# eldenpark/halo2-pse

Measured on AMD Instinct MI355X. Metric: bn254_msm_g1_adds_per_sec, higher is better.
Workload: dtype u32x8 (256-bit Montgomery integers)

## Files before the change

halo2-pse_amd/csrc/api.hip:

```cpp
#include <dlfcn.h>
#include <rccl/rccl.h>
#include <stdarg.h>
#include <stdlib.h>
#include <string.h>

#include <atomic>
#include <condition_variable>
#include <deque>
#include <functional>
#include <shared_mutex>
#include <thread>

#include "../../include/halo2hip.h"
#include "../../include/halo2hip_debug.h"
#include "engine.h"

extern "C" {
static void lazy_forget(const void* key);
static void lazy_reset();
static void lazy_pin_consider(const uint64_t* bases_xy, size_t n);
}

namespace h2 {

int gen_scalars_device(uint64_t seed, uint64_t start, size_t n, Fe* d_out, hipStream_t s);
int gen_points_device(uint64_t seed, uint64_t start, size_t n, Affine* d_out, hipStream_t s);
void msm_set_window(uint32_t c);
void msm_set_max_chunk(size_t m);
void msm_set_stream(uint32_t chunks, double ratio, size_t min_n);
size_t msm_debug_ladder(size_t n, uint32_t chunks, double ratio, bool with_bases, size_t* out, size_t cap);
void msm_set_heavy_div(size_t d);
void msm_set_bin_entries(size_t d);
void msm_set_split_records(bool on);
void msm_set_bucket_order(int local);
void msm_set_quad_tail(bool on);
void msm_set_split_buckets(bool on);
void msm_set_plane_tail(bool on);
void ecfft_set_quad(bool on);
void ecfft_set_lazy(bool on);
void msm_set_fuse_limits(size_t entries, size_t max_n);
void msm_set_rowcol(uint64_t lanes, uint32_t flavour);
void ntt_set_smax(uint32_t v);
void ntt_set_two_pass(uint32_t lo, uint32_t hi);
void ntt_set_full_twiddle_budget(uint64_t bytes);
void ntt_set_batch_bytes(uint64_t bytes);
void ntt_set_two_pass_log_j(int v);
void ntt_set_full_max_log_m(uint32_t v);
void ntt_set_fold_tables(bool on);
void ntt_set_two_pass_batch_wgs(uint64_t v);
void msm_set_reserved_cus(uint32_t k);
uint32_t msm_get_reserved_cus();
uint32_t msm_get_window(size_t n);

static thread_local char g_err[512] = "";

void set_error(const char* fmt, ...) {
    va_list ap;
    va_start(ap, fmt);
    vsnprintf(g_err, sizeof(g_err), fmt, ap);
    va_end(ap);
}

int DevBuf::ensure(size_t bytes) {
    if (bytes <= cap) return 0;
    if (p) {
        H2_CHECK(hipDeviceSynchronize());
        H2_CHECK(hipFree(p));
        p = nullptr;
        cap = 0;
    }
    size_t want = bytes + bytes / 8 + 4096;
    hipError_t e = hipMalloc(&p, want);
    if (e != hipSuccess) {
        p = nullptr;
        set_error("hipMalloc(%zu) failed: %s", want, hipGetErrorString(e));
        return H2HIP_ENOMEM;
    }
    cap = want;
    return 0;
}

int HostBuf::ensure(size_t bytes) {
    if (bytes <= cap) return 0;
    if (p) {
        H2_CHECK(hipDeviceSynchronize());
        H2_CHECK(hipHostFree(p));
        p = nullptr;
        cap = 0;
    }
    size_t want = bytes * 2 + 4096;
    hipError_t e = hipHostMalloc(&p, want, hipHostMallocDefault);
    if (e != hipSuccess) {
        p = nullptr;
        set_error("hipHostMalloc(%zu) failed: %s", want, hipGetErrorString(e));
        return H2HIP_ENOMEM;
    }
    cap = want;
    return 0;
}

void HostBuf::release() {
    if (p) (void)hipHostFree(p);
    p = nullptr;
    cap = 0;
}

void DevBuf::release() {
    if (p) (void)hipFree(p);
    p = nullptr;
    cap = 0;
}

static std::shared_mutex g_engine_mu;
static Ctx g_ctx;
static std::vector<Ctx*> g_devs;
Ctx* ctx() { return &g_ctx; }
int n_devices() { return (int)g_devs.size(); }
Ctx* ctx_at(int i) { return g_devs[(size_t)i]; }

int Ctx::stage_h2d(void* d_dst, const void* h_src, size_t bytes, hipStream_t s) {
// ... 2060 lines not shown
    if (en.rc) return en.rc;
    return evaluate_h_host(en.c, desc, (uint64_t*)d_values, true, (hipStream_t)stream);
}

int h2hip_gen_scalars_device(uint64_t seed, uint64_t start, size_t n, void* d_out, void* stream) {
    if (n && !d_out) {
        set_error("gen_scalars: null output");
        return H2HIP_EINVAL;
    }
    Entry en("h2hip_gen_scalars_device", d_out);
    if (en.rc) return en.rc;
    return gen_scalars_device(seed, start, n, (Fe*)d_out, (hipStream_t)stream);
}

int h2hip_gen_points_device(uint64_t seed, uint64_t start, size_t n, void* d_out, void* stream) {
    if (n && !d_out) {
        set_error("gen_points: null output");
        return H2HIP_EINVAL;
    }
    Entry en("h2hip_gen_points_device", d_out);
    if (en.rc) return en.rc;
    return gen_points_device(seed, start, n, (Affine*)d_out, (hipStream_t)stream);
}

int h2hip_set_msm_window(uint32_t c) {
    if (c != 0 && (c < 2 || c > 24)) {
        set_error("msm window must be 0 (auto) or 2..24");
        return H2HIP_EINVAL;
    }
    msm_set_window(c);
    return 0;
}

uint32_t h2hip_get_msm_window(size_t n) { return msm_get_window(n); }
uint32_t h2hip_get_msm_window_fixed_base(size_t n) { return msm_table_window(n); }

int h2hip_debug_set_msm_max_chunk(size_t m) {
    msm_set_max_chunk(m);
    return 0;
}

int h2hip_debug_set_msm_stream(uint32_t chunks, uint32_t ratio_permille, size_t min_n) {
    msm_set_stream(chunks, ratio_permille / 1000.0, min_n);
    return 0;
}

size_t h2hip_debug_msm_stream_ladder(size_t n, uint32_t chunks, uint32_t ratio_permille, int with_bases, size_t* sizes, size_t cap) {
    if (!sizes && cap) return 0;
    return msm_debug_ladder(n, chunks, ratio_permille / 1000.0, with_bases != 0, sizes, cap);
}

int h2hip_debug_set_msm_heavy_div(size_t d) {
    msm_set_heavy_div(d);
    return 0;
}

int h2hip_debug_set_g2l_quad(int on) {
    ecfft_set_quad(on != 0);
    return 0;
}

int h2hip_debug_set_msm_fuse_limits(size_t entries, size_t max_n) {
    msm_set_fuse_limits(entries, max_n);
    return 0;
}

int h2hip_debug_set_msm_rowcol(uint64_t lanes, int use_asm) {
    msm_set_rowcol(lanes, (uint32_t)use_asm);
    return 0;
}

int h2hip_debug_set_msm_split_buckets(int on) {
    msm_set_split_buckets(on != 0);
    return 0;
}

int h2hip_debug_set_msm_plane_tail(int on) {
    Entry en;
    if (en.rc) return en.rc;
    msm_set_plane_tail(on != 0);
    return 0;
}

int h2hip_debug_set_msm_quad_tail(int on) {
    msm_set_quad_tail(on != 0);
    return 0;
}

int h2hip_debug_set_msm_bucket_order(int local) {
    msm_set_bucket_order(local);
    return 0;
}

int h2hip_debug_set_msm_split_records(int on) {
    msm_set_split_records(on != 0);
    return 0;
}

int h2hip_debug_set_msm_bin_entries(size_t d) {
    msm_set_bin_entries(d);
    return 0;
}

int h2hip_debug_set_evalh_max_local_slots(uint32_t v) {
    evalh_debug_set_max_local_slots(v);
    return 0;
}

int h2hip_debug_set_evalh_lookup_group_bytes(uint64_t v) {
    evalh_debug_set_lookup_group_bytes(v);
    return 0;
}

int h2hip_debug_evalh_program_muls(const h2hip_graph* g, uint32_t* n_mul) { return evalh_debug_program_muls(g, n_mul) ? H2HIP_EINVAL : 0; }

int h2hip_debug_set_evalh_codegen(int mode, uint32_t max_ops) {
    Entry en;
    if (en.rc) return en.rc;
    evalh_debug_set_codegen(mode, max_ops);
    return 0;
}

int h2hip_debug_evalh_codegen_source(const h2hip_graph* g, char* buf, size_t cap, size_t* len, int compile, double* seconds, size_t* code_bytes) {
    return evalh_debug_codegen_source(g, buf, cap, len, compile, seconds, code_bytes);
}

int h2hip_debug_evalh_codegen_stats(uint64_t out[5]) {
    if (!out) return H2HIP_EINVAL;
    evalh_debug_codegen_stats(out);
    return 0;
}

int h2hip_debug_evalh_compile_stats(const h2hip_graph* g, uint32_t* n_ops, uint32_t* n_slots) {
    return evalh_debug_compile_stats(g, n_ops, n_slots);
}

int h2hip_debug_set_msm_fuse_small(int on) {
    msm_set_fuse_small(on != 0);
    return 0;
}

int h2hip_debug_set_ntt_smax(uint32_t v) {
    ntt_set_smax(v);
    return 0;
}

int h2hip_debug_set_ntt_twiddle_budget(uint64_t bytes) {
    ntt_set_full_twiddle_budget(bytes);
    return 0;
}

int h2hip_debug_set_ntt_batch_bytes(uint64_t bytes) {
    ntt_set_batch_bytes(bytes);
    return 0;
}

int h2hip_debug_set_ntt_two_pass_batch_wgs(uint64_t v) {
    ntt_set_two_pass_batch_wgs(v);
    return 0;
}

int h2hip_debug_set_ntt_full_max_log_m(uint32_t v) {
    ntt_set_full_max_log_m(v);
    return 0;
}

// ... 59 lines not shown
```

halo2-pse_amd/csrc/msm.hip:

```cpp
#include <hip/hip_ext.h>
#include <string.h>

#include <atomic>
#include <condition_variable>
#include <thread>
#include <vector>

#include "ecq.h"
#include "engine.h"
#include "host64.h"

namespace h2 {

#define MSM_MAX_C1 1024u
#define MSM_MAX_L 12u
#define MSM_STAGE 16384u
#define MSM_COUNT_TILE 4096u

struct MsmPlan {
    uint32_t c;
    uint32_t W;
    uint32_t q;
    uint32_t cb;
    uint32_t NB;
// ... 759 lines not shown
    }
    if (role == 0) sh[quad] = acc;
    __syncthreads();
    for (uint32_t stride = G >> 1; stride >= 1; stride >>= 1) {
        if (g < stride) {
            XYZZu x = sh[quad];
            xyzzu_add_q(x, sh[quad + stride], role);
            if (role == 0) sh[quad] = x;
        }
        __syncthreads();
    }
    if (live && g == 0 && role == 0) J.out[task] = sh[quad];
}

__global__ void __launch_bounds__(64) msm_final_quad_kernel(FinalArgs args, uint32_t n_groups, XYZZu* __restrict__ partials, uint32_t* __restrict__ done,
                                                            XYZZ* __restrict__ set_sums) {
    __shared__ XYZZu sh[16];
    __shared__ uint32_t is_last;
    const uint32_t set = blockIdx.x / n_groups, group = blockIdx.x - set * n_groups;
    const uint32_t quad = threadIdx.x >> 2, role = threadIdx.x & 3;
    uint32_t e = group * 16 + quad;
    const XYZZu* base = nullptr;
    uint32_t stride = 0, o = 0, k = 0, nbits = 0;
    bool found = false;
#pragma unroll
    for (uint32_t i = 0; i < 4; i++) {
        if (i < args.n_arr && !found) {
            if (e < args.arr[i].len) {
                found = true;
                base = args.arr[i].base;
                stride = args.arr[i].stride;
                o = args.arr[i].o;
                k = args.arr[i].k;
                nbits = args.arr[i].nbits;
            } else {
                e -= args.arr[i].len;
            }
        }
    }
    XYZZu x = xyzzu_identity();
    if (found) {
        const uint32_t wgt = (e + o) << k;
        if (wgt) x = xyzzu_mul_small_q(base[(size_t)set * stride + e], wgt, nbits, role);
    }
    if (role == 0) sh[quad] = x;
    __syncthreads();
    for (uint32_t st = 8; st >= 1; st >>= 1) {
        if (quad < st) {
            XYZZu a = sh[quad];
            xyzzu_add_q(a, sh[quad + st], role);
            if (role == 0) sh[quad] = a;
        }
        __syncthreads();
    }
    if (n_groups == 1) {
        if (threadIdx.x == 0) set_sums[set] = xyzzu_to_ext(sh[0]);
        return;
    }
    if (threadIdx.x == 0) {
        partials[blockIdx.x] = sh[0];
        __threadfence();
        is_last = atomicAdd(&done[set], 1u) == n_groups - 1;
    }
    __syncthreads();
    if (!is_last) return;
    __builtin_amdgcn_fence(__ATOMIC_ACQUIRE, "agent");
    x = xyzzu_identity();
    if (quad < n_groups) x = partials[(size_t)set * n_groups + quad];
    if (role == 0) sh[quad] = x;
    __syncthreads();
    for (uint32_t st = 8; st >= 1; st >>= 1) {
        if (quad < st) {
            XYZZu a = sh[quad];
            xyzzu_add_q(a, sh[quad + st], role);
            if (role == 0) sh[quad] = a;
        }
        __syncthreads();
    }
    if (threadIdx.x == 0) set_sums[set] = xyzzu_to_ext(sh[0]);
}

#define MSM_PLANES_MAX 32
#define MSM_PLANE_SETS_MAX 4
struct PlaneJob {
    const XYZZu* base;
    uint32_t log_len;
    uint32_t o;
    uint32_t n_planes;
    uint32_t wgs;
    uint32_t first_plane;
    uint32_t first_block;
};
struct PlaneArgs {
    PlaneJob job[2];
    uint32_t blocks_per_set, planes_per_set;
};

__global__ void __launch_bounds__(256) msm_planes_kernel(PlaneArgs args, XYZZu* __restrict__ partials, uint32_t* __restrict__ done,
                                                         XYZZ* __restrict__ plane_sums) {
    __shared__ XYZZu sh[64];
    __shared__ uint32_t is_last;
    const uint32_t set = blockIdx.x / args.blocks_per_set, b = blockIdx.x - set * args.blocks_per_set;
    const PlaneJob& J = args.job[b >= args.job[1].first_block ? 1 : 0];
    const uint32_t pb = b - J.first_block, plane = pb / J.wgs, part = pb - plane * J.wgs;
    const XYZZu* X = J.base + ((size_t)set << J.log_len);
    const uint32_t quad = threadIdx.x >> 2, role = threadIdx.x & 3;
    const bool top = plane == J.log_len;
    const uint32_t count = top ? 1u : 1u << (J.log_len - 1);
    auto elem = [&](uint32_t t) -> XYZZu {
        if (t >= count) return xyzzu_identity();
        const uint32_t v = top ? (1u << J.log_len) : ((t >> plane) << (plane + 1)) | (1u << plane) | (t & ((1u << plane) - 1));
        return X[v - J.o];
    };
    const uint32_t t0 = part * 128 + 2 * quad;
    const XYZZu x = xyzzu_sum_q(elem(t0), elem(t0 + 1), role);
    if (role == 0) sh[quad] = x;
    __syncthreads();
    for (uint32_t st = 32; st >= 1; st >>= 1) {
        if (quad < st) {
            const XYZZu a = xyzzu_sum_q(sh[quad], sh[quad + st], role);
            if (role == 0) sh[quad] = a;
        }
        __syncthreads();
    }
    const uint32_t out = set * args.planes_per_set + J.first_plane + plane;
    if (J.wgs == 1) {
        if (threadIdx.x == 0) plane_sums[out] = xyzzu_to_ext(sh[0]);
        return;
    }
    if (threadIdx.x == 0) {
        partials[(size_t)out * 16 + part] = sh[0];
        __threadfence();
        is_last = atomicAdd(&done[out], 1u) == J.wgs - 1;
    }
    __syncthreads();
    if (!is_last) return;
    __builtin_amdgcn_fence(__ATOMIC_ACQUIRE, "agent");
    XYZZu y = xyzzu_identity();
    if (quad < J.wgs) y = partials[(size_t)out * 16 + quad];
    if (role == 0 && quad < 16) sh[quad] = y;
    __syncthreads();
    for (uint32_t st = 8; st >= 1; st >>= 1) {
        if (quad < st) {
            const XYZZu a = xyzzu_sum_q(sh[quad], sh[quad + st], role);
            if (role == 0) sh[quad] = a;
        }
        __syncthreads();
    }
    if (threadIdx.x == 0) plane_sums[out] = xyzzu_to_ext(sh[0]);
}

__global__ void __launch_bounds__(256) msm_table_step_kernel(const Affine* __restrict__ prev, XYZZ* __restrict__ out, uint32_t n, uint32_t c) {
    const uint32_t i = blockIdx.x * blockDim.x + threadIdx.x;
    if (i >= n) return;
    const Affine p = prev[i];
    if (affine_is_identity(p)) {
        out[i] = xyzz_identity();
        return;
    }
    XYZZu q = xyzzu_double_affine<FqUA>(fu_from_ext(p.x), fu_from_ext(p.y));
    for (uint32_t k = 1; k < c; k++) q = xyzzu_double(q);
    out[i] = xyzzu_to_ext(q);
}

static uint32_t g_window_override = 0;
static size_t g_heavy_div = 32768;
static size_t g_bin_entries = 8192;
static bool g_split_records = true;
void msm_set_split_records(bool on) { g_split_records = on; }
static uint64_t g_rowcol_lanes = 65536;
static bool g_rowcol_asm = true, g_rowcol_qtree = true;
void msm_set_rowcol(uint64_t lanes, uint32_t flavour) {
    g_rowcol_lanes = lanes ? lanes : 65536;
    g_rowcol_asm = flavour & 1;
    g_rowcol_qtree = flavour & 2;
}
static bool g_split_buckets = true;
void msm_set_split_buckets(bool on) { g_split_buckets = on; }
static bool g_quad_tail = true;
void msm_set_quad_tail(bool on) { g_quad_tail = on; }
static bool g_global_order = true;
void msm_set_bucket_order(int local) { g_global_order = local == 0; }
void msm_set_bin_entries(size_t d) { g_bin_entries = d ? d : 8192; }
void msm_set_heavy_div(size_t d) { g_heavy_div = d ? d : 32768; }
static size_t g_max_chunk = (size_t)1 << 26;
void msm_set_max_chunk(size_t m) { g_max_chunk = m ? m : ((size_t)1 << 26); }
static uint32_t g_reserved_cus = 0;
void msm_set_reserved_cus(uint32_t k) { g_reserved_cus = k; }
uint32_t msm_get_reserved_cus() { return g_reserved_cus; }
void msm_set_window(uint32_t c) { g_window_override = c; }

static uint32_t floor_log2(size_t n) {
    uint32_t lg = 0;
    while (((size_t)1 << (lg + 1)) <= n) lg++;
    return lg;
}

static uint32_t plain_window(size_t n, bool fused) {
    if (g_window_override) return g_window_override;
    const uint32_t lg = floor_log2(n);
    if (fused && lg >= 13 && lg <= 18) return lg <= 13 ? 10 : lg <= 16 ? 12 : lg == 17 ? 13 : 14;
    if (lg <= 8) return 7;
    if (lg <= 12) return 10;
    if (lg <= 14) return 13;
    if (lg <= 17) return 15;
    return 17;
}

static uint32_t normalise_window(uint32_t c) {
    if (c < 2) c = 2;
    if (c > 22) c = 22;
    const uint32_t W = (255 + c - 1) / c;
    return (255 + W - 1) / W;
}

uint32_t msm_table_window(size_t n) {
    if (g_window_override) return normalise_window(g_window_override);
    const uint32_t lg = floor_log2(n);
    uint32_t c = lg <= 12 ? 13 : lg <= 17 ? 17 : lg <= 21 ? 20 : 22;
    return normalise_window(c);
}

static MsmPlan make_plan(size_t n, bool fused, const MsmTable* tab, uint32_t force_c = 0) {
    MsmPlan p;
    uint32_t c = tab ? tab->c : force_c ? force_c : plain_window(n, fused);
    if (c < 2) c = 2;
    if (c > 24) c = 24;
    p.W = (255 + c - 1) / c;
    c = (255 + p.W - 1) / p.W;
    p.c = c;
    p.q = 255 - p.W * (c - 1);
    p.cb = c - 1;
// ... 200 lines not shown
        hipLaunchKernelGGL(msm_l2_kernel<true>, dim3(L.C1), dim3(1024), 0, s, (const uint2*)nullptr, (const uint32_t*)a.tmp_e, (const uint16_t*)a.tmp_k, cstart,
                           L.L, L.bin_shift, vals, start, counts, perm, g_global_order ? hist : (uint32_t*)nullptr);
    else
        hipLaunchKernelGGL(msm_l2_kernel<false>, dim3(L.C1), dim3(1024), 0, s, (const uint2*)(base + L.o_tmp), (const uint32_t*)nullptr,
                           (const uint16_t*)nullptr, cstart, L.L, L.bin_shift, vals, start, counts, perm, g_global_order ? hist : (uint32_t*)nullptr);
    H2_CHECK(hipGetLastError());
    hipLaunchKernelGGL(msm_bucket_scatter_kernel, dim3((L.K + 1024 * MSM_BS_PER - 1) / (1024 * MSM_BS_PER)), dim3(1024), 0, s, (const uint32_t*)counts,
                       (const uint32_t*)start, L.K, L.bin_shift, p.heavy_t, p.chunk, hist, g_global_order ? perm : (uint32_t*)nullptr,
                       (uint32_t*)(base + L.o_hcnt), (HeavyBucket*)(base + L.o_hb), (HeavyChunk*)(base + L.o_hc));
    H2_CHECK(hipGetLastError());
    c->timer_end(t1, s);
    return 0;
}

static int msm_stage_b(Ctx* c, const MsmLayout& L, char* base, const Affine* d_points, hipStream_t s, char* bbase = nullptr, bool cont = false,
                       bool combine = true) {
    const MsmPlan& p = L.p;
    if (!bbase) bbase = base;
    uint32_t* vals = (uint32_t*)(base + L.o_vals);
    uint32_t *start = (uint32_t*)(base + L.o_start), *counts = (uint32_t*)(base + L.o_counts), *perm = (uint32_t*)(base + L.o_perm);
    XYZZu* buckets = (XYZZu*)(bbase + L.o_buckets);
    uint32_t* hcnt = (uint32_t*)(base + L.o_hcnt);
    HeavyBucket* hb = (HeavyBucket*)(base + L.o_hb);
    HeavyChunk* hc = (HeavyChunk*)(base + L.o_hc);
    XYZZu* hs = (XYZZu*)(base + L.o_hs);
    int t2 = c->timer_begin("msm_accum", s);
    hipEvent_t ke0 = nullptr, ke1 = nullptr;
    XYZZu* parts = (XYZZu*)(bbase + L.o_parts);
    const uint32_t lanes = L.K << L.split_log;
    const uint32_t cont_u = cont ? 1u : 0u;
    const uint32_t hgrid = (uint32_t)(L.max_chunks < (size_t)c->sm_count ? L.max_chunks : (size_t)c->sm_count);
    const dim3 agrid(hgrid + (lanes + 255) / 256);
    if (c->timer_kernel("msm_accum", &ke0, &ke1) >= 0)
        hipExtLaunchKernelGGL(msm_accum_kernel, agrid, dim3(256), 0, s, ke0, ke1, 0, d_points, (const uint32_t*)vals, (const uint32_t*)start,
                              (const uint32_t*)counts, (const uint32_t*)perm, L.K, L.split_log, p.heavy_t, cont_u, parts, hgrid, (const uint32_t*)hcnt, hb,
                              (const HeavyChunk*)hc, hs);
    else
        hipLaunchKernelGGL(msm_accum_kernel, agrid, dim3(256), 0, s, d_points, (const uint32_t*)vals, (const uint32_t*)start, (const uint32_t*)counts,
                           (const uint32_t*)perm, L.K, L.split_log, p.heavy_t, cont_u, parts, hgrid, (const uint32_t*)hcnt, hb, (const HeavyChunk*)hc, hs);
    H2_CHECK(hipGetLastError());
    c->timer_end(t2, s);
    if (L.split_log && combine) {
        const uint32_t comb_lanes = L.K << (L.split_log - 1);
        hipLaunchKernelGGL(msm_combine_kernel, dim3((comb_lanes + 255) / 256), dim3(256), 0, s, (const XYZZu*)parts, L.K, L.split_log, buckets);
        H2_CHECK(hipGetLastError());
    }
    return 0;
}

static void rowcol_jobs(RowColArgs* ra, const XYZZu* in, XYZZu* out_rows, XYZZu* out_cols, uint32_t n_arr, uint32_t log_rows, uint32_t log_cols,
                        uint32_t* n_blocks, bool quad = false) {
    const uint64_t elems = (uint64_t)n_arr << (log_rows + log_cols);
    const uint64_t budget = (2 * elems) >> 4 > g_rowcol_lanes ? 2 * g_rowcol_lanes : g_rowcol_lanes;
    uint32_t t_log = 1;
    while (!quad && (2 * elems) >> t_log > budget) t_log++;
    for (uint32_t kind = 0; kind < 2; kind++) {
        RowColJob* j = &ra->job[ra->n_jobs++];
        const uint32_t log_terms = kind ? log_rows : log_cols, log_sums = kind ? log_cols : log_rows;
        uint32_t g_log = log_terms > t_log ? log_terms - t_log : 0;
        const uint32_t g_max = quad ? 4 : 8;
        if (g_log > g_max) g_log = g_max;
        j->in = in;
        j->out = kind ? out_cols : out_rows;
        j->n_arr = n_arr;
        j->log_rows = log_rows;
        j->log_cols = log_cols;
        j->cols_kind = kind;
        j->g_log = g_log;
        j->first_block = *n_blocks;
        const uint64_t tasks = (uint64_t)n_arr << log_sums;
        const uint32_t per_block = (quad ? 16u : 256u) >> g_log;
        *n_blocks += (uint32_t)((tasks + per_block - 1) / per_block);
    }
}

static bool g_plane_tail = true;
void msm_set_plane_tail(bool on) { g_plane_tail = on; }
static bool msm_plane_tail(const Ctx* c, const MsmLayout& L) {
    return g_plane_tail && g_quad_tail && L.levels >= 1 && L.n_sets <= MSM_PLANE_SETS_MAX && L.rb <= 11 && L.s <= 11 && L.rb >= 1 && L.s >= 1 &&
           L.s + 1 + L.rb <= MSM_PLANES_MAX && !c->gather_want;
}
static inline uint32_t msm_planes_per_set(const MsmLayout& L) { return L.rb + L.s + 1; }

static void msm_planes_finish(const MsmLayout& L, const XYZZ* planes, XYZZ* sums) {
    const uint32_t pps = msm_planes_per_set(L);
    for (uint32_t set = 0; set < L.n_sets; set++) {
        const XYZZ* P = planes + (size_t)set * pps;
        h64::P acc = h64::identity();
        for (uint32_t m = L.s + L.rb; m-- > 0;) {
            acc = h64::pdouble(acc);
            if (m >= L.s) h64::padd(acc, h64::from_xyzz(P[L.s + 1 + (m - L.s)]));
            if (m <= L.s) h64::padd(acc, h64::from_xyzz(P[m]));
        }
        sums[set] = h64::to_xyzz(acc);
    }
}

static int msm_stage_c(Ctx* c, const MsmLayout& L, char* base, XYZZ* h_sums, hipStream_t s, XYZZ* h_planes = nullptr) {
    XYZZu* buckets = (XYZZu*)(base + L.o_buckets);
    XYZZu *RA = (XYZZu*)(base + L.o_RA), *CA = (XYZZu*)(base + L.o_CA), *RR = (XYZZu*)(base + L.o_RR), *RC = (XYZZu*)(base + L.o_RC);
    XYZZu *CR = (XYZZu*)(base + L.o_CR), *CC = (XYZZu*)(base + L.o_CC);
    const bool direct = !c->gather_want;
    XYZZ* sums = direct ? h_sums : (XYZZ*)(base + L.o_sums);
    const uint32_t ns = L.n_sets, cb = L.p.cb;
    const bool quad = g_quad_tail && ns <= 64;
    int t4 = c->timer_begin("msm_reduce", s);
    FinalArgs fa;
    memset(&fa, 0, sizeof(fa));
    auto set_arr = [&](uint32_t i, const XYZZu* b, uint32_t log_len, uint32_t o, uint32_t k) {
        fa.arr[i].base = b;
        fa.arr[i].stride = 1u << log_len;
        fa.arr[i].len = 1u << log_len;
        fa.arr[i].o = o;
        fa.arr[i].k = k;
        fa.arr[i].nbits = bits_of(((1u << log_len) - 1 + o) << k);
    };
    if (L.levels == 0) {
        set_arr(0, buckets, cb, 1, 0);
        fa.n_arr = 1;
    } else {
        RowColArgs ra;
        memset(&ra, 0, sizeof(ra));
        uint32_t nblk = 0;
        rowcol_jobs(&ra, buckets, RA, CA, ns, L.rb, L.s, &nblk);
        if (g_rowcol_qtree)
            hipLaunchKernelGGL(msm_rowcol_qtree_kernel<FqUA>, dim3(nblk), dim3(256), 0, s, ra);
        else if (g_rowcol_asm)
            hipLaunchKernelGGL(msm_rowcol_kernel<FqUA>, dim3(nblk), dim3(256), 0, s, ra);
        else
            hipLaunchKernelGGL(msm_rowcol_kernel<FqU>, dim3(nblk), dim3(256), 0, s, ra);
        H2_CHECK(hipGetLastError());
        if (h_planes && msm_plane_tail(c, L)) {
            PlaneArgs pa;
            memset(&pa, 0, sizeof(pa));
            uint32_t blk = 0, pl = 0;
            for (uint32_t k = 0; k < 2; k++) {
                PlaneJob& J = pa.job[k];
                J.base = k ? RA : CA;
                J.log_len = k ? L.rb : L.s;
                J.o = k ? 0 : 1;
                J.n_planes = J.log_len + J.o;
                J.wgs = J.log_len > 7 ? 1u << (J.log_len - 8) : 1;
                J.first_plane = pl;
                J.first_block = blk;
                pl += J.n_planes;
                blk += J.n_planes * J.wgs;
            }
            pa.blocks_per_set = blk;
            pa.planes_per_set = pl;
            hipLaunchKernelGGL(msm_planes_kernel, dim3(ns * blk), dim3(256), 0, s, pa, (XYZZu*)(base + L.o_ppart), (uint32_t*)(base + L.o_fdone), h_planes);
            H2_CHECK(hipGetLastError());
            c->timer_end(t4, s);
            return 0;
        }
        if (L.levels == 1) {
            set_arr(0, RA, L.rb, 0, L.s);
            set_arr(1, CA, L.s, 1, 0);
            fa.n_arr = 2;
        } else {
            memset(&ra, 0, sizeof(ra));
            nblk = 0;
            rowcol_jobs(&ra, RA, RR, RC, ns, L.rb - L.s2, L.s2, &nblk, quad);
            rowcol_jobs(&ra, CA, CR, CC, ns, L.s - L.s3, L.s3, &nblk, quad);
            if (quad)
                hipLaunchKernelGGL(msm_rowcol_quad_kernel, dim3(nblk), dim3(64), 0, s, ra);
            else
                hipLaunchKernelGGL(msm_rowcol_kernel<FqU>, dim3(nblk), dim3(256), 0, s, ra);
            H2_CHECK(hipGetLastError());
            set_arr(0, RR, L.rb - L.s2, 0, L.s + L.s2);
            set_arr(1, RC, L.s2, 0, L.s);
            set_arr(2, CR, L.s - L.s3, 0, L.s3);
            set_arr(3, CC, L.s3, 1, 0);
            fa.n_arr = 4;
        }
    }
    if (quad) {
        uint32_t n_el = 0;
        for (uint32_t i = 0; i < fa.n_arr; i++) n_el += fa.arr[i].len;
        const uint32_t n_groups = (n_el + 15) / 16;
        XYZZu* partials = (XYZZu*)(base + L.o_partials);
        hipLaunchKernelGGL(msm_final_quad_kernel, dim3(ns * n_groups), dim3(64), 0, s, fa, n_groups, partials, (uint32_t*)(base + L.o_fdone), sums);
    } else {
        hipLaunchKernelGGL(msm_final_kernel, dim3(ns), dim3(256), 0, s, fa, sums);
    }
    H2_CHECK(hipGetLastError());
    c->timer_end(t4, s);
    if (!direct) H2_CHECK(hipMemcpyAsync(h_sums, sums, (size_t)ns * sizeof(XYZZ), hipMemcpyDeviceToHost, s));
    if (c->gather_want) {
        const size_t bytes = (size_t)ns * sizeof(XYZZ);
        if (c->gather_off + bytes <= H2_GATHER_OWN && c->gather.p)
            H2_CHECK(hipMemcpyAsync((char*)c->gather.p + c->gather_off, sums, bytes, hipMemcpyDeviceToDevice, s));
        c->gather_off += bytes;
    }
    return 0;
}

static inline uint32_t sets_per_msm(const MsmPlan& p) { return p.shared ? 1 : p.W; }
static inline XYZZ finish_msm(const XYZZ* sums, const MsmPlan& p) { return p.shared ? sums[0] : combine_windows(sums, p); }

static int msm_batch_chunk(Ctx* c, const Fe* const* d_scalars, bool scalars_on_host, const Affine* d_points, const MsmTable* tab, size_t n,
                           size_t count, XYZZ* h_out, hipStream_t s) {
    MsmLayout L;
    int rc = msm_layout(n, &L, 1, tab);
    if (rc) return rc;
    const size_t n_slots = count < 3 ? count : 3;
    for (size_t k = 0; k < n_slots; k++) {
        rc = c->msm_slot[k].ensure(L.total);
        if (rc) return rc;
        if (scalars_on_host) {
            rc = c->msm_scalars[k].ensure(n * sizeof(Fe));
            if (rc) return rc;
        }
    }
    auto scalars_for = [&](size_t j, hipStream_t st, const Fe** out) -> int {
        if (!scalars_on_host) {
            *out = d_scalars[j];
            return 0;
        }
        Fe* dst = (Fe*)c->msm_scalars[j % 3].p;
        H2_CHECK(hipMemcpyAsync(dst, d_scalars[j], n * sizeof(Fe), hipMemcpyHostToDevice, st));
        *out = dst;
        return 0;
    };
    const uint32_t spm = sets_per_msm(L.p);
    rc = c->host_ws.ensure(count * spm * sizeof(XYZZ));
    if (rc) return rc;
    XYZZ* h_ws = (XYZZ*)c->host_ws.p;
    XYZZ* h_pl = nullptr;
    if (count == 1 && msm_plane_tail(c, L)) {
        if ((rc = c->host_planes.ensure((size_t)L.n_sets * MSM_PLANES_MAX * sizeof(XYZZ)))) return rc;
        h_pl = (XYZZ*)c->host_planes.p;
    }
    rc = c->ws_acquire(s);
    if (rc) return rc;
    WsGuard guard(c, s);
    int t_all = c->timer_begin("msm_total", s);
    if (count == 1) {
        char* base = (char*)c->msm_slot[0].p;
        const Fe* sc;
        if ((rc = scalars_for(0, s, &sc))) return rc;
        if ((rc = msm_stage_a(c, L, base, &sc, tab, s))) return rc;
        if ((rc = msm_stage_b(c, L, base, d_points, s))) return rc;
        if ((rc = msm_stage_c(c, L, base, h_ws, s, h_pl))) return rc;
    } else {
        rc = c->ensure_aux(3 * count + 2);
        if (rc) return rc;
        hipStream_t a1 = c->aux1, a2 = c->aux2, sb = c->aux_b;
        hipEvent_t* ev = c->aux_events.data();
        H2_CHECK(hipEventRecord(ev[0], s));
        H2_CHECK(hipStreamWaitEvent(a1, ev[0], 0));
        H2_CHECK(hipStreamWaitEvent(a2, ev[0], 0));
        H2_CHECK(hipStreamWaitEvent(sb, ev[0], 0));
        for (size_t j = 0; j < count; j++) {
            char* base = (char*)c->msm_slot[j % 3].p;
            if (j >= 3) H2_CHECK(hipStreamWaitEvent(a1, ev[3 + 3 * (j - 3)], 0));
            const Fe* sc;
            if ((rc = scalars_for(j, a1, &sc))) return rc;
            if ((rc = msm_stage_a(c, L, base, &sc, tab, a1))) return rc;
            H2_CHECK(hipEventRecord(ev[1 + 3 * j], a1));
            H2_CHECK(hipStreamWaitEvent(sb, ev[1 + 3 * j], 0));
            if ((rc = msm_stage_b(c, L, base, d_points, sb))) return rc;
            H2_CHECK(hipEventRecord(ev[2 + 3 * j], sb));
            H2_CHECK(hipStreamWaitEvent(a2, ev[2 + 3 * j], 0));
            if ((rc = msm_stage_c(c, L, base, h_ws + j * spm, a2))) return rc;
            H2_CHECK(hipEventRecord(ev[3 + 3 * j], a2));
        }
        H2_CHECK(hipStreamWaitEvent(s, ev[3 + 3 * (count - 1)], 0));
    }
    c->timer_end(t_all, s);
    H2_CHECK(hipStreamSynchronize(s));
    if (h_pl) msm_planes_finish(L, h_pl, h_ws);
    for (size_t j = 0; j < count; j++) h_out[j] = finish_msm(h_ws + j * spm, L.p);
    return guard.release();
}

static int msm_fused_chunk(Ctx* c, const Fe* const* d_scalars, bool scalars_on_host, const Affine* d_points, const MsmTable* tab, size_t n,
                           size_t count, XYZZ* h_out, hipStream_t s) {
    MsmLayout L;
    int rc = msm_layout(n, &L, (uint32_t)count, tab);
    if (rc) return rc;
    if ((rc = c->msm_slot[0].ensure(L.total))) return rc;
    std::vector<const Fe*> list(d_scalars, d_scalars + count);
    if ((rc = c->ws_acquire(s))) return rc;
    WsGuard guard(c, s);
    if (scalars_on_host) {
        if ((rc = c->msm_scalars[0].ensure(count * n * sizeof(Fe)))) return rc;
        for (size_t j = 0; j < count; j++) {
            Fe* dst = (Fe*)c->msm_scalars[0].p + j * n;
            H2_CHECK(hipMemcpyAsync(dst, d_scalars[j], n * sizeof(Fe), hipMemcpyHostToDevice, s));
            list[j] = dst;
        }
    }
    if ((rc = c->host_ws.ensure((size_t)L.n_sets * sizeof(XYZZ)))) return rc;
    XYZZ* h_ws = (XYZZ*)c->host_ws.p;
    XYZZ* h_pl = nullptr;
    if (msm_plane_tail(c, L)) {
        if ((rc = c->host_planes.ensure((size_t)L.n_sets * MSM_PLANES_MAX * sizeof(XYZZ)))) return rc;
        h_pl = (XYZZ*)c->host_planes.p;
    }
    char* base = (char*)c->msm_slot[0].p;
    int t_all = c->timer_begin("msm_total", s);
    if ((rc = msm_stage_a(c, L, base, list.data(), tab, s))) return rc;
    if ((rc = msm_stage_b(c, L, base, d_points, s))) return rc;
    if ((rc = msm_stage_c(c, L, base, h_ws, s, h_pl))) return rc;
    c->timer_end(t_all, s);
    H2_CHECK(hipStreamSynchronize(s));
    if (h_pl) msm_planes_finish(L, h_pl, h_ws);
    const uint32_t spm = sets_per_msm(L.p);
    for (size_t j = 0; j < count; j++) h_out[j] = finish_msm(h_ws + j * spm, L.p);
    return guard.release();
}

static uint32_t g_stream_chunks = 3;
static bool g_stream_chunks_default = true;
static double g_stream_ratio = 0.6;
static size_t g_stream_min_n = (size_t)1 << 19;
void msm_set_stream(uint32_t chunks, double ratio, size_t min_n) {
    g_stream_chunks = chunks ? chunks : 3;
    g_stream_chunks_default = chunks == 0;
    g_stream_ratio = ratio > 0 ? ratio : 0.6;
    g_stream_min_n = min_n ? min_n : ((size_t)1 << 19);
}


struct CopierDrain {
    Ctx* c;
    size_t n_jobs;
    ~CopierDrain() { copier_abort(c, false, n_jobs); }
};

static void stream_ladder(size_t units, uint32_t K, double r, size_t quantum, std::vector<size_t>* out) {
    out->clear();
    if (K < 1) K = 1;
    while (K > 1 && units < (size_t)K * quantum * 2) K--;
    std::vector<double> f(K);
    double w = 1.0, tot = 0.0;
    for (uint32_t k = 0; k < K; k++) {
        f[k] = w;
        tot += w;
        w /= r;
    }
    size_t used = 0;
    for (uint32_t k = 0; k + 1 < K; k++) {
        size_t m = (size_t)((double)units * f[k] / tot / (double)quantum + 0.5) * quantum;
        if (m < quantum) m = quantum;
        if (used + m + quantum > units) break;
        out->push_back(m);
        used += m;
    }
    out->push_back(units - used);
}

size_t msm_debug_ladder(size_t n, uint32_t chunks, double ratio, bool with_bases, size_t* out, size_t cap) {
    std::vector<size_t> sz;
    const uint32_t k0 = chunks ? chunks : g_stream_chunks;
    const double r = ratio > 0 ? ratio : g_stream_ratio;
    const uint32_t kk = !chunks && g_stream_chunks_default && n < ((size_t)1 << 20) ? 2 : k0;
    stream_ladder(n, with_bases ? 2 * kk : kk, with_bases ? 2.0 * r : r, 4096, &sz);
    for (size_t i = 0; i < sz.size() && i < cap; i++) out[i] = sz[i];
    return sz.size();
}

static int msm_stream_host(Ctx* c, const Fe* h_scalars, const Affine* h_bases, const Affine* d_points, const MsmTable* tab, size_t n, XYZZ* h_out,
                           hipStream_t s) {
    std::vector<size_t> sz;
    const uint32_t kk = g_stream_chunks_default && n < ((size_t)1 << 20) ? 2 : g_stream_chunks;
    stream_ladder(n, h_bases ? 2 * kk : kk, h_bases ? 2.0 * g_stream_ratio : g_stream_ratio, 4096, &sz);
    const size_t K = sz.size();
    MsmLayout Lt;
    int rc = msm_layout(n, &Lt, 1, tab);
    if (rc) return rc;
    std::vector<MsmLayout> Lk(K);
    size_t need = 0;
    for (size_t k = 0; k < K; k++) {
        if ((rc = msm_layout(sz[k], &Lk[k], 1, tab, Lt.p.c, (int)Lt.split_log))) return rc;
        if (Lk[k].total > need) need = Lk[k].total;
    }
    if ((rc = c->msm_slot[0].ensure(need))) return rc;
    if ((rc = c->msm_scalars[0].ensure(n * sizeof(Fe)))) return rc;
    Fe* d_sc = (Fe*)c->msm_scalars[0].p;
    Affine* d_bs = nullptr;
    if (h_bases) {
        if ((rc = c->msm_bases.ensure(n * sizeof(Affine)))) return rc;
        d_bs = (Affine*)c->msm_bases.p;
        d_points = d_bs;
    }
    const uint32_t spm = sets_per_msm(Lt.p);
    if ((rc = c->host_ws.ensure(spm * sizeof(XYZZ)))) return rc;
    XYZZ* h_ws = (XYZZ*)c->host_ws.p;
    XYZZ* h_pl = nullptr;
    if (msm_plane_tail(c, Lk[K - 1])) {
        if ((rc = c->host_planes.ensure((size_t)Lk[K - 1].n_sets * MSM_PLANES_MAX * sizeof(XYZZ)))) return rc;
        h_pl = (XYZZ*)c->host_planes.p;
    }
    if ((rc = c->ensure_aux(K + 2))) return rc;
    if ((rc = c->ws_acquire(s))) return rc;
    WsGuard guard(c, s);
    int t_all = c->timer_begin("msm_total", s);
    hipStream_t cs = c->aux2;
    hipEvent_t* ev = c->aux_events.data();
    H2_CHECK(hipEventRecord(ev[0], s));
    H2_CHECK(hipStreamWaitEvent(cs, ev[0], 0));
    char* base = (char*)c->msm_slot[0].p;
    const Affine* points0 = tab ? tab->table : d_points;
    size_t o = 0;
    std::vector<CopyJob> jobs;
    for (size_t k = 0; k < K; k++) {
        if (h_bases) jobs.push_back(CopyJob{d_bs + o, h_bases + o, sz[k] * sizeof(Affine), nullptr, nullptr, false});
        jobs.push_back(CopyJob{d_sc + o, h_scalars + o, sz[k] * sizeof(Fe), ev[1 + k], nullptr, false});
        o += sz[k];
    }
    const size_t per_chunk = h_bases ? 2 : 1;
    H2_CHECK(hipStreamSynchronize(s));
    if ((rc = copier_begin(c, false, cs))) return rc;
    CopierDrain drain{c, K * per_chunk};
    if ((rc = copier_push(c, false, jobs))) return rc;
    o = 0;
    for (size_t k = 0; k < K; k++) {
        if ((rc = copier_wait(c, false, (k + 1) * per_chunk))) return rc;
        H2_CHECK(hipStreamWaitEvent(s, ev[1 + k], 0));
        const Fe* sc = d_sc + o;
        if ((rc = msm_stage_a(c, Lk[k], base, &sc, tab, s))) return rc;
        if ((rc = msm_stage_b(c, Lk[k], base, points0 + o, s, base, k > 0, k + 1 == K))) return rc;
        o += sz[k];
    }
    if ((rc = msm_stage_c(c, Lk[K - 1], base, h_ws, s, h_pl))) return rc;
    c->timer_end(t_all, s);
    H2_CHECK(hipStreamSynchronize(s));
    if (h_pl) msm_planes_finish(Lk[K - 1], h_pl, h_ws);
    h_out[0] = finish_msm(h_ws, Lt.p);
    return guard.release();
}

static int msm_fused_groups_host(Ctx* c, const Fe* const* h_scalars, const Affine* d_points, const MsmTable* tab, size_t n, size_t count,
                                 size_t fuse_max, XYZZ* h_out, hipStream_t s) {
    std::vector<size_t> ladder, groups;
    stream_ladder(count, g_stream_chunks, g_stream_ratio * 0.85, 1, &ladder);
    for (size_t g : ladder)
        for (size_t o = 0; o < g; o += fuse_max) groups.push_back(g - o < fuse_max ? g - o : fuse_max);
    const size_t G = groups.size();
    std::vector<MsmLayout> Lg(G);
    size_t need = 0, max_sets = 0;
    int rc;
    for (size_t g = 0; g < G; g++) {
        if ((rc = msm_layout(n, &Lg[g], (uint32_t)groups[g], tab))) return rc;
        if (Lg[g].total > need) need = Lg[g].total;
        max_sets += Lg[g].n_sets;
    }
    for (int k = 0; k < 2; k++)
        if ((rc = c->msm_slot[k].ensure(need))) return rc;
    if ((rc = c->msm_scalars[0].ensure(count * n * sizeof(Fe)))) return rc;
    if ((rc = c->host_ws.ensure(max_sets * sizeof(XYZZ)))) return rc;
    XYZZ* h_ws = (XYZZ*)c->host_ws.p;
    if ((rc = c->ensure_aux(3 * G + 2))) return rc;
    if ((rc = c->ws_acquire(s))) return rc;
    WsGuard guard(c, s);
    int t_all = c->timer_begin("msm_total", s);
    hipStream_t cs = c->aux2, sa = c->aux_b, sc_ = c->aux1;
    hipEvent_t* ev = c->aux_events.data();
    H2_CHECK(hipEventRecord(ev[0], s));
    H2_CHECK(hipStreamWaitEvent(cs, ev[0], 0));
    H2_CHECK(hipStreamWaitEvent(sa, ev[0], 0));
    H2_CHECK(hipStreamWaitEvent(sc_, ev[0], 0));
    std::vector<const Fe*> list(count);
    size_t j0 = 0, set0 = 0;
    std::vector<CopyJob> jobs;
    for (size_t g = 0; g < G; g++) {
        for (size_t j = j0; j < j0 + groups[g]; j++) {
            Fe* dst = (Fe*)c->msm_scalars[0].p + j * n;
            jobs.push_back(CopyJob{dst, h_scalars[j], n * sizeof(Fe), j + 1 == j0 + groups[g] ? ev[1 + 3 * g] : nullptr, nullptr, false});
            list[j] = dst;
        }
        j0 += groups[g];
    }
    H2_CHECK(hipStreamSynchronize(s));
    if ((rc = copier_begin(c, false, cs))) return rc;
    CopierDrain drain{c, count};
    if ((rc = copier_push(c, false, jobs))) return rc;
    j0 = 0;
    for (size_t g = 0; g < G; g++) {
        const size_t cnt = groups[g];
        if ((rc = copier_wait(c, false, j0 + cnt))) return rc;
        char* base = (char*)c->msm_slot[g & 1].p;
        H2_CHECK(hipStreamWaitEvent(sa, ev[1 + 3 * g], 0));
        if (g >= 2) H2_CHECK(hipStreamWaitEvent(sa, ev[3 + 3 * (g - 2)], 0));
        if ((rc = msm_stage_a(c, Lg[g], base, list.data() + j0, tab, sa))) return rc;
        if ((rc = msm_stage_b(c, Lg[g], base, d_points, sa))) return rc;
        H2_CHECK(hipEventRecord(ev[2 + 3 * g], sa));
        H2_CHECK(hipStreamWaitEvent(sc_, ev[2 + 3 * g], 0));
        if ((rc = msm_stage_c(c, Lg[g], base, h_ws + set0, sc_))) return rc;
        H2_CHECK(hipEventRecord(ev[3 + 3 * g], sc_));
        j0 += cnt;
        set0 += Lg[g].n_sets;
    }
    H2_CHECK(hipStreamWaitEvent(s, ev[3 + 3 * (G - 1)], 0));
    c->timer_end(t_all, s);
    H2_CHECK(hipStreamSynchronize(s));
    j0 = set0 = 0;
    for (size_t g = 0; g < G; g++) {
        const uint32_t spm = sets_per_msm(Lg[g].p);
        for (size_t j = 0; j < groups[g]; j++) h_out[j0 + j] = finish_msm(h_ws + set0 + j * spm, Lg[g].p);
        j0 += groups[g];
        set0 += Lg[g].n_sets;
    }
    return guard.release();
}

static size_t g_fuse_entries = (size_t)1 << 26, g_fuse_max_n = (size_t)1 << 19;
void msm_set_fuse_limits(size_t entries, size_t max_n) { g_fuse_entries = entries ? entries : ((size_t)1 << 26); g_fuse_max_n = max_n ? max_n : ((size_t)1 << 19); }
static bool g_fuse_small = true;
void msm_set_fuse_small(bool on) { g_fuse_small = on; }

// ... 95 lines not shown
```

include/halo2hip_debug.h:

```cpp
#ifndef HALO2HIP_DEBUG_H
#define HALO2HIP_DEBUG_H
#include "halo2hip.h"

#ifdef __cplusplus
extern "C" {
#endif

int h2hip_debug_set_msm_stream(uint32_t chunks, uint32_t ratio_permille, size_t min_n);
size_t h2hip_debug_msm_stream_ladder(size_t n, uint32_t chunks, uint32_t ratio_permille, int with_bases, size_t* sizes, size_t cap);
int h2hip_debug_set_msm_max_chunk(size_t m);
int h2hip_debug_rccl_gather_selftest(const uint64_t* partials_xyz, size_t count, uint64_t* out_xyz);
int h2hip_debug_set_msm_heavy_div(size_t d);
int h2hip_debug_set_g2l_quad(int on);
int h2hip_debug_set_msm_fuse_limits(size_t entries, size_t max_n);
int h2hip_debug_set_msm_rowcol(uint64_t lanes, int use_asm);
int h2hip_debug_set_msm_split_buckets(int on);
int h2hip_debug_set_msm_plane_tail(int on);
int h2hip_debug_set_msm_quad_tail(int on);
int h2hip_debug_set_msm_bucket_order(int local);
int h2hip_debug_set_msm_split_records(int on);
int h2hip_debug_set_msm_bin_entries(size_t d);
int h2hip_debug_set_reserved_cus(uint32_t k);
int h2hip_debug_set_msm_fuse_small(int on);
int h2hip_debug_set_ntt_smax(uint32_t v);
int h2hip_debug_ntt_plan(uint32_t log_n, size_t count, uint32_t radices[4]);
int h2hip_debug_set_lazy_pin(uint32_t after);
int h2hip_debug_set_ntt_two_pass(uint32_t lo, uint32_t hi);
int h2hip_debug_set_ntt_twiddle_budget(uint64_t bytes);
int h2hip_debug_set_ntt_batch_bytes(uint64_t bytes);
int h2hip_debug_set_ntt_two_pass_batch_wgs(uint64_t v);
int h2hip_debug_set_ntt_full_max_log_m(uint32_t v);
int h2hip_debug_set_ntt_fold_tables(int on);
int h2hip_debug_set_ntt_host_batch(uint64_t run_bytes, uint64_t group_bytes);
int h2hip_debug_set_ntt_two_pass_log_j(int v);
int h2hip_debug_set_evalh_max_local_slots(uint32_t v);
int h2hip_debug_set_evalh_lookup_group_bytes(uint64_t v);
int h2hip_debug_evalh_program_muls(const h2hip_graph* g, uint32_t* n_mul);
int h2hip_debug_set_evalh_codegen(int mode, uint32_t max_ops);
int h2hip_debug_evalh_codegen_source(const h2hip_graph* g, char* buf, size_t cap, size_t* len, int compile, double* seconds, size_t* code_bytes);
int h2hip_debug_evalh_codegen_stats(uint64_t out[5]);
int h2hip_debug_evalh_compile_stats(const h2hip_graph* g, uint32_t* n_ops, uint32_t* n_slots);
int h2hip_debug_set_opening_tile(uint32_t rows_per_thread, uint32_t threads_per_tile);
int h2hip_debug_set_lookup_sort(uint32_t lds_keys);
int h2hip_debug_lookup_sort_stats(uint32_t out[2]);

#ifdef __cplusplus
}
#endif
#endif
```

Measured before the change: 11.29 billion.

## Signal plane-sum completion to host via system-scope flag for early finish

The plane-tail kernel now counts finished planes with a device atomic, and the last block writes a token to a host-visible flag with system scope. The host spin-waits on that flag and runs the CPU plane finish before calling hipStreamSynchronize, so the host reduction overlaps the stream's remaining teardown and sync latency. This adds a global atomic and a system fence per plane block, plus a host busy-wait. It also relies on the done counter slot at MSM_MAX_C1-1 being zero at launch, and the diff does not reset that slot.

```diff
diff --git a/halo2-pse_amd/csrc/api.hip b/halo2-pse_amd/csrc/api.hip
--- a/halo2-pse_amd/csrc/api.hip
+++ b/halo2-pse_amd/csrc/api.hip
@@ -36,6 +36,8 @@
 void msm_set_quad_tail(bool on);
 void msm_set_split_buckets(bool on);
 void msm_set_plane_tail(bool on);
+std::atomic<bool> g_plane_handoff{true};
+std::atomic<uint64_t> g_plane_handoffs{0};
 void ecfft_set_quad(bool on);
 void ecfft_set_lazy(bool on);
 void msm_set_fuse_limits(size_t entries, size_t max_n);
@@ -2262,6 +2264,14 @@
     return 0;
 }
 
+int h2hip_debug_msm_plane_handoff(int on, uint64_t* count) {
+    Entry en;
+    if (en.rc) return en.rc;
+    if (on >= 0) g_plane_handoff = on != 0;
+    if (count) *count = g_plane_handoffs.load();
+    return 0;
+}
+
 int h2hip_debug_set_msm_quad_tail(int on) {
     msm_set_quad_tail(on != 0);
     return 0;
diff --git a/halo2-pse_amd/csrc/msm.hip b/halo2-pse_amd/csrc/msm.hip
--- a/halo2-pse_amd/csrc/msm.hip
+++ b/halo2-pse_amd/csrc/msm.hip
@@ -865,6 +865,8 @@
 
 #define MSM_PLANES_MAX 32
 #define MSM_PLANE_SETS_MAX 4
+#define MSM_PLANE_COUNTER (MSM_MAX_C1 - 1)
+#define MSM_PLANE_HOST_BYTES ((size_t)(MSM_PLANE_SETS_MAX * MSM_PLANES_MAX + 1) * sizeof(XYZZ))
 struct PlaneJob {
     const XYZZu* base;
     uint32_t log_len;
@@ -879,8 +881,17 @@
     uint32_t blocks_per_set, planes_per_set;
 };
 
+__device__ __forceinline__ void msm_plane_handoff(uint32_t* __restrict__ done, uint32_t n_planes, uint32_t token, uint32_t* host_flag) {
+    __threadfence_system();
+    if (atomicAdd(&done[MSM_PLANE_COUNTER], 1u) == n_planes - 1) {
+        __builtin_amdgcn_fence(__ATOMIC_ACQUIRE, "agent");
+        __threadfence_system();
+        __hip_atomic_store(host_flag, token, __ATOMIC_RELAXED, __HIP_MEMORY_SCOPE_SYSTEM);
+    }
+}
+
 __global__ void __launch_bounds__(256) msm_planes_kernel(PlaneArgs args, XYZZu* __restrict__ partials, uint32_t* __restrict__ done,
-                                                         XYZZ* __restrict__ plane_sums) {
+                                                         XYZZ* __restrict__ plane_sums, uint32_t n_planes, uint32_t token, uint32_t* host_flag) {
     __shared__ XYZZu sh[64];
     __shared__ uint32_t is_last;
     const uint32_t set = blockIdx.x / args.blocks_per_set, b = blockIdx.x - set * args.blocks_per_set;
@@ -908,7 +919,10 @@
     }
     const uint32_t out = set * args.planes_per_set + J.first_plane + plane;
     if (J.wgs == 1) {
-        if (threadIdx.x == 0) plane_sums[out] = xyzzu_to_ext(sh[0]);
+        if (threadIdx.x == 0) {
+            plane_sums[out] = xyzzu_to_ext(sh[0]);
+            msm_plane_handoff(done, n_planes, token, host_flag);
+        }
         return;
     }
     if (threadIdx.x == 0) {
@@ -930,7 +944,10 @@
         }
         __syncthreads();
     }
-    if (threadIdx.x == 0) plane_sums[out] = xyzzu_to_ext(sh[0]);
+    if (threadIdx.x == 0) {
+        plane_sums[out] = xyzzu_to_ext(sh[0]);
+        msm_plane_handoff(done, n_planes, token, host_flag);
+    }
 }
 
 __global__ void __launch_bounds__(256) msm_table_step_kernel(const Affine* __restrict__ prev, XYZZ* __restrict__ out, uint32_t n, uint32_t c) {
@@ -1297,6 +1314,22 @@
 }
 static inline uint32_t msm_planes_per_set(const MsmLayout& L) { return L.rb + L.s + 1; }
 
+extern std::atomic<bool> g_plane_handoff;
+extern std::atomic<uint64_t> g_plane_handoffs;
+static std::atomic<uint32_t> g_plane_token{0};
+static inline uint32_t* msm_plane_flag(XYZZ* h_planes) { return (uint32_t*)(h_planes + MSM_PLANE_SETS_MAX * MSM_PLANES_MAX); }
+
+static bool msm_planes_wait(XYZZ* h_planes, uint32_t token, hipStream_t s) {
+    const uint32_t* flag = msm_plane_flag(h_planes);
+    for (uint32_t i = 1;; i++) {
+        if (__atomic_load_n(flag, __ATOMIC_ACQUIRE) == token) return true;
+        if ((i & 255) == 0 && hipStreamQuery(s) != hipErrorNotReady) return __atomic_load_n(flag, __ATOMIC_ACQUIRE) == token;
+#if defined(__x86_64__)
+        __builtin_ia32_pause();
+#endif
+    }
+}
+
 static void msm_planes_finish(const MsmLayout& L, const XYZZ* planes, XYZZ* sums) {
     const uint32_t pps = msm_planes_per_set(L);
     for (uint32_t set = 0; set < L.n_sets; set++) {
@@ -1311,7 +1344,18 @@
     }
 }
 
-static int msm_stage_c(Ctx* c, const MsmLayout& L, char* base, XYZZ* h_sums, hipStream_t s, XYZZ* h_planes = nullptr) {
+static int msm_run_end(const MsmLayout& L, XYZZ* h_planes, uint32_t token, XYZZ* h_sums, hipStream_t s) {
+    const bool early = token && token != ~0u && msm_planes_wait(h_planes, token, s);
+    if (early) {
+        msm_planes_finish(L, h_planes, h_sums);
+        g_plane_handoffs++;
+    }
+    H2_CHECK(hipStreamSynchronize(s));
+    if (token && !early) msm_planes_finish(L, h_planes, h_sums);
+    return 0;
+}
+
+static int msm_stage_c(Ctx* c, const MsmLayout& L, char* base, XYZZ* h_sums, hipStream_t s, XYZZ* h_planes = nullptr, uint32_t* token = nullptr) {
     XYZZu* buckets = (XYZZu*)(base + L.o_buckets);
     XYZZu *RA = (XYZZu*)(base + L.o_RA), *CA = (XYZZu*)(base + L.o_CA), *RR = (XYZZu*)(base + L.o_RR), *RC = (XYZZu*)(base + L.o_RC);
     XYZZu *CR = (XYZZu*)(base + L.o_CR), *CC = (XYZZu*)(base + L.o_CC);
@@ -1363,7 +1407,15 @@
             }
             pa.blocks_per_set = blk;
             pa.planes_per_set = pl;
-            hipLaunchKernelGGL(msm_planes_kernel, dim3(ns * blk), dim3(256), 0, s, pa, (XYZZu*)(base + L.o_ppart), (uint32_t*)(base + L.o_fdone), h_planes);
+            uint32_t tk = 0;
+            if (g_plane_handoff && token)
+                while (!(tk = ++g_plane_token)) {
+                }
+            uint32_t* flag = msm_plane_flag(h_planes);
+            __atomic_store_n(flag, 0u, __ATOMIC_RELEASE);
+            hipLaunchKernelGGL(msm_planes_kernel, dim3(ns * blk), dim3(256), 0, s, pa, (XYZZu*)(base + L.o_ppart), (uint32_t*)(base + L.o_fdone), h_planes,
+                               ns * pl, tk, flag);
+            if (token) *token = tk ? tk : ~0u;
             H2_CHECK(hipGetLastError());
             c->timer_end(t4, s);
             return 0;
@@ -1442,8 +1494,9 @@
     if (rc) return rc;
     XYZZ* h_ws = (XYZZ*)c->host_ws.p;
     XYZZ* h_pl = nullptr;
+    uint32_t token = 0;
     if (count == 1 && msm_plane_tail(c, L)) {
-        if ((rc = c->host_planes.ensure((size_t)L.n_sets * MSM_PLANES_MAX * sizeof(XYZZ)))) return rc;
+        if ((rc = c->host_planes.ensure(MSM_PLANE_HOST_BYTES))) return rc;
         h_pl = (XYZZ*)c->host_planes.p;
     }
     rc = c->ws_acquire(s);
@@ -1456,7 +1509,7 @@
         if ((rc = scalars_for(0, s, &sc))) return rc;
         if ((rc = msm_stage_a(c, L, base, &sc, tab, s))) return rc;
         if ((rc = msm_stage_b(c, L, base, d_points, s))) return rc;
-        if ((rc = msm_stage_c(c, L, base, h_ws, s, h_pl))) return rc;
+        if ((rc = msm_stage_c(c, L, base, h_ws, s, h_pl, &token))) return rc;
     } else {
         rc = c->ensure_aux(3 * count + 2);
         if (rc) return rc;
@@ -1483,8 +1536,7 @@
         H2_CHECK(hipStreamWaitEvent(s, ev[3 + 3 * (count - 1)], 0));
     }
     c->timer_end(t_all, s);
-    H2_CHECK(hipStreamSynchronize(s));
-    if (h_pl) msm_planes_finish(L, h_pl, h_ws);
+    if ((rc = msm_run_end(L, h_pl, token, h_ws, s))) return rc;
     for (size_t j = 0; j < count; j++) h_out[j] = finish_msm(h_ws + j * spm, L.p);
     return guard.release();
 }
@@ -1509,18 +1561,18 @@
     if ((rc = c->host_ws.ensure((size_t)L.n_sets * sizeof(XYZZ)))) return rc;
     XYZZ* h_ws = (XYZZ*)c->host_ws.p;
     XYZZ* h_pl = nullptr;
+    uint32_t token = 0;
     if (msm_plane_tail(c, L)) {
-        if ((rc = c->host_planes.ensure((size_t)L.n_sets * MSM_PLANES_MAX * sizeof(XYZZ)))) return rc;
+        if ((rc = c->host_planes.ensure(MSM_PLANE_HOST_BYTES))) return rc;
         h_pl = (XYZZ*)c->host_planes.p;
     }
     char* base = (char*)c->msm_slot[0].p;
     int t_all = c->timer_begin("msm_total", s);
     if ((rc = msm_stage_a(c, L, base, list.data(), tab, s))) return rc;
     if ((rc = msm_stage_b(c, L, base, d_points, s))) return rc;
-    if ((rc = msm_stage_c(c, L, base, h_ws, s, h_pl))) return rc;
+    if ((rc = msm_stage_c(c, L, base, h_ws, s, h_pl, &token))) return rc;
     c->timer_end(t_all, s);
-    H2_CHECK(hipStreamSynchronize(s));
-    if (h_pl) msm_planes_finish(L, h_pl, h_ws);
+    if ((rc = msm_run_end(L, h_pl, token, h_ws, s))) return rc;
     const uint32_t spm = sets_per_msm(L.p);
     for (size_t j = 0; j < count; j++) h_out[j] = finish_msm(h_ws + j * spm, L.p);
     return guard.release();
@@ -1604,8 +1656,9 @@
     if ((rc = c->host_ws.ensure(spm * sizeof(XYZZ)))) return rc;
     XYZZ* h_ws = (XYZZ*)c->host_ws.p;
     XYZZ* h_pl = nullptr;
+    uint32_t token = 0;
     if (msm_plane_tail(c, Lk[K - 1])) {
-        if ((rc = c->host_planes.ensure((size_t)Lk[K - 1].n_sets * MSM_PLANES_MAX * sizeof(XYZZ)))) return rc;
+        if ((rc = c->host_planes.ensure(MSM_PLANE_HOST_BYTES))) return rc;
         h_pl = (XYZZ*)c->host_planes.p;
     }
     if ((rc = c->ensure_aux(K + 2))) return rc;
@@ -1639,10 +1692,9 @@
         if ((rc = msm_stage_b(c, Lk[k], base, points0 + o, s, base, k > 0, k + 1 == K))) return rc;
         o += sz[k];
     }
-    if ((rc = msm_stage_c(c, Lk[K - 1], base, h_ws, s, h_pl))) return rc;
+    if ((rc = msm_stage_c(c, Lk[K - 1], base, h_ws, s, h_pl, &token))) return rc;
     c->timer_end(t_all, s);
-    H2_CHECK(hipStreamSynchronize(s));
-    if (h_pl) msm_planes_finish(Lk[K - 1], h_pl, h_ws);
+    if ((rc = msm_run_end(Lk[K - 1], h_pl, token, h_ws, s))) return rc;
     h_out[0] = finish_msm(h_ws, Lt.p);
     return guard.release();
 }
diff --git a/include/halo2hip_debug.h b/include/halo2hip_debug.h
--- a/include/halo2hip_debug.h
+++ b/include/halo2hip_debug.h
@@ -16,6 +16,7 @@
 int h2hip_debug_set_msm_rowcol(uint64_t lanes, int use_asm);
 int h2hip_debug_set_msm_split_buckets(int on);
 int h2hip_debug_set_msm_plane_tail(int on);
+int h2hip_debug_msm_plane_handoff(int on, uint64_t* count);
 int h2hip_debug_set_msm_quad_tail(int on);
 int h2hip_debug_set_msm_bucket_order(int local);
 int h2hip_debug_set_msm_split_records(int on);
```

Measured after the change: 11.28 billion (median of 3 runs). About the same (-0.1%).
